# meg89/bevfusion_multimodal_3d_object_detection

Hardware: AMD Instinct MI355X
Metric: BEV frames/sec (6-cam+LiDAR, 128x128 BEV) (higher is better)
Workload: dtype fp32; 1 GPU; camera+LiDAR, 6x900x1600 images + 35k-point sweep, BEV 128x128; batch_per_gpu=8, parallelism=replicas x1, conv_kernels=wino, weights=random-init (synthetic, seeded), launch=eager, mode=inference forward -> 5 head tensors

## Files before the change

bevfusion_multimodal_3d_object_detection_amd/csrc/conv_split.hip:

```cpp
#include "conv_common.h"

#include <cmath>

namespace {

typedef __bf16 bf16x4 __attribute__((ext_vector_type(4)));
typedef unsigned u32x2 __attribute__((ext_vector_type(2)));

__device__ __forceinline__ void split3(const f32x4 v, u32x2& hi, u32x2& mid, u32x2& lo) {
  const bf16x4 h = __builtin_convertvector(v, bf16x4);
  const f32x4 r1 = v - __builtin_convertvector(h, f32x4);
  const bf16x4 m = __builtin_convertvector(r1, bf16x4);
  const f32x4 r2 = r1 - __builtin_convertvector(m, f32x4);
  const bf16x4 l = __builtin_convertvector(r2, bf16x4);
  hi = __builtin_bit_cast(u32x2, h);
  mid = __builtin_bit_cast(u32x2, m);
  lo = __builtin_bit_cast(u32x2, l);
}

__global__ __launch_bounds__(256) void split_weights(const float* __restrict__ w, __bf16* __restrict__ out, long long n) {
  const long long i = blockIdx.x * 256ll + threadIdx.x;
  if (i >= n) return;
  const float x = w[i];
  const __bf16 h = (__bf16)x;
  const float r1 = x - (float)h;
  const __bf16 m = (__bf16)r1;
  const float r2 = r1 - (float)m;
  out[i] = h;
  out[n + i] = m;
  out[2 * n + i] = (__bf16)r2;
}

template <int BM, int BN, int WM, int WN>
__device__ __forceinline__ void bound_epilogue(const ConvArgs& p, f32x16 (&acc)[WM / 32][WN / 32], const int m0, const int n0,
                                               const int m_hi, const int wm, const int wn, const int lane, const float* norms) {
  constexpr int MI = WM / 32, NI = WN / 32;
  const int h = lane >> 5, l31 = lane & 31;
  const int row_base = wm * WM + 4 * h, n_base = n0 + wn * WN;
  const int group = m0 / p.rows_per_group;
  const bool fast = (m0 + BM <= m_hi) && ((m0 + BM - 1) / p.rows_per_group == group);
  float na[MI][16];
#pragma unroll
  for (int mi = 0; mi < MI; ++mi)
#pragma unroll
    for (int r = 0; r < 16; ++r) na[mi][r] = norms[row_base + mi * 32 + (r & 3) + 8 * (r >> 2)];
  unsigned fmask[MI];
#pragma unroll
  for (int mi = 0; mi < MI; ++mi) fmask[mi] = 0u;
#pragma unroll
  for (int ni = 0; ni < NI; ++ni) {
    const int n = n_base + ni * 32 + l31;
    const bool nok = n < p.Cout;
    const int nc = nok ? n : p.Cout - 1;
    float sc, sh;
    conv_scale_shift(p, nc, sc, sh);
    const float g = p.bound_g[nc];
    const float thr = fast ? __uint_as_float(__hip_atomic_load(&p.colmax[(size_t)group * p.Cout + nc], __ATOMIC_RELAXED, __HIP_MEMORY_SCOPE_AGENT)) : 0.f;
    float lbmax = 0.f;
#pragma unroll
    for (int mi = 0; mi < MI; ++mi) {
#pragma unroll
      for (int r = 0; r < 16; ++r) {
        const float val = fmaf(acc[mi][ni][r], sc, sh);
        const float eps = fmaf(na[mi][r], g, fabsf(val) * 0x1p-21f);
        const float ub = val + eps;
        const float lb = fabsf(val) < __builtin_inff() ? val - eps : 0.f;
        if (fast) {
          lbmax = fmaxf(lbmax, lb);
          if (p.flag && !(ub < thr) && !(ub <= 0.f)) fmask[mi] |= 1u << r;
        } else {
          const int m = m0 + row_base + mi * 32 + (r & 3) + 8 * (r >> 2);
          if (m < m_hi && nok) {
            uint32_t* const t = &p.colmax[(size_t)(m / p.rows_per_group) * p.Cout + n];
            const float th = __uint_as_float(__hip_atomic_load(t, __ATOMIC_RELAXED, __HIP_MEMORY_SCOPE_AGENT));
            if (lb > th) atomicMax(t, __float_as_uint(lb));
            if (p.flag && !(ub < th) && !(ub <= 0.f)) fmask[mi] |= 1u << r;
          }
        }
      }
    }
    if (fast) {
      lbmax = fmaxf(lbmax, __shfl_xor(lbmax, 32));
      if (h == 0 && nok && lbmax > thr) atomicMax(&p.colmax[(size_t)group * p.Cout + n], __float_as_uint(lbmax));
    }
  }
  if (!p.flag) return;
#pragma unroll
  for (int mi = 0; mi < MI; ++mi) {
    unsigned f = fmask[mi];
#pragma unroll
    for (int d = 1; d < 32; d <<= 1) f |= (unsigned)__shfl_xor((int)f, d);
    const int m = m0 + row_base + mi * 32 + (l31 & 3) + 8 * ((l31 >> 2) & 3);
    if (l31 < 16 && ((f >> l31) & 1u) && m < m_hi) p.flag[m] = 1;
  }
}

template <int BM, int BN, int WM, int WN, int NPL = 3, bool BOUND = false>
__global__ __launch_bounds__(256) void conv_split(const ConvArgs p) {
  static_assert(NPL == 3 || (NPL == 2 && BOUND), "two planes are the bound pass");
  constexpr int WAVES_N = BN / WN;
  constexpr int MI = WM / 32, NI = WN / 32;
  constexpr int AP = BM / 32, BPJ = BN / 64;
  static_assert((BM / WM) * (BN / WN) == 4, "4 waves per workgroup");
  constexpr int A_PLANE = BM * 64, B_PLANE = BN * 64, B_BASE = NPL * A_PLANE;
  extern __shared__ __attribute__((aligned(16))) float lds[];
  char* const ldsb = reinterpret_cast<char*>(lds);

  const int sid = xcd_remap(blockIdx.x, gridDim.x);
  const int tm = (sid / p.tilesN) * (BOUND ? p.tm_stride : 1), tn = sid % p.tilesN;
  const int m_hi = p.M;
  const int tid = threadIdx.x, lane = tid & 63;
  const int wave = __builtin_amdgcn_readfirstlane(tid >> 6);
  const int wm = wave / WAVES_N, wn = wave % WAVES_N;
  const int m0 = tm * BM, n0 = tn * BN;

  const int chunk = tid & 7, srow = tid >> 3;
  ConvAWalker<4, AP> aw;
  aw.init(p, m0 + srow, m_hi, chunk);
  const int bq = tid & 3, brow = tid >> 2;
  unsigned b_voff[BPJ];
#pragma unroll
  for (int j = 0; j < BPJ; ++j) {
    const int n = n0 + brow + 64 * j;
    b_voff[j] = n < p.Cout ? (unsigned)(((size_t)n * p.K) * 2 + bq * 16) : kOob;
  }
  const size_t plane_elems = (size_t)p.Cout * p.K;
  const __bf16* const wb = static_cast<const __bf16*>(p.w);
  const __amdgpu_buffer_rsrc_t rsrcB0 = buf_rsrc(wb), rsrcB1 = buf_rsrc(wb + plane_elems), rsrcB2 = buf_rsrc(wb + 2 * plane_elems);

  f32x4 ra[AP];
  u32x4 rb[NPL][BPJ];
  float ssq[AP];
#pragma unroll
  for (int j = 0; j < AP; ++j) ssq[j] = 0.f;
  auto load_tile = [&](int kstep) {
    aw.load(p, ra);
#pragma unroll
    for (int j = 0; j < BPJ; ++j) {
      rb[0][j] = __builtin_amdgcn_raw_buffer_load_b128(rsrcB0, b_voff[j], (unsigned)kstep * 64u, 0);
      rb[1][j] = __builtin_amdgcn_raw_buffer_load_b128(rsrcB1, b_voff[j], (unsigned)kstep * 64u, 0);
      if constexpr (NPL == 3) rb[2][j] = __builtin_amdgcn_raw_buffer_load_b128(rsrcB2, b_voff[j], (unsigned)kstep * 64u, 0);
    }
  };

  const int a_wr = srow * 64 + (((chunk >> 1) ^ ((srow >> 1) & 3)) << 4) + (chunk & 1) * 8;
  const int b_wr = B_BASE + brow * 64 + ((bq ^ ((brow >> 1) & 3)) << 4);
  const int h = lane >> 5, l31 = lane & 31;
  int a_rd[2], b_rd[2];
#pragma unroll
  for (int g = 0; g < 2; ++g) {
    a_rd[g] = (wm * WM + l31) * 64 + (((2 * g + h) ^ ((l31 >> 1) & 3)) << 4);
    b_rd[g] = B_BASE + (wn * WN + l31) * 64 + (((2 * g + h) ^ ((l31 >> 1) & 3)) << 4);
  }
  auto store_tile = [&]() {
#pragma unroll
    for (int j = 0; j < AP; ++j) {
      u32x2 hi, mid, lo;
      split3(ra[j], hi, mid, lo);
      *reinterpret_cast<u32x2*>(ldsb + a_wr + j * 2048) = hi;
      *reinterpret_cast<u32x2*>(ldsb + a_wr + j * 2048 + A_PLANE) = mid;
      if constexpr (NPL == 3) *reinterpret_cast<u32x2*>(ldsb + a_wr + j * 2048 + 2 * A_PLANE) = lo;
      if constexpr (BOUND) ssq[j] = fmaf(ra[j][0], ra[j][0], fmaf(ra[j][1], ra[j][1], fmaf(ra[j][2], ra[j][2], fmaf(ra[j][3], ra[j][3], ssq[j]))));
    }
#pragma unroll
    for (int pl = 0; pl < NPL; ++pl)
#pragma unroll
      for (int j = 0; j < BPJ; ++j) *reinterpret_cast<u32x4*>(ldsb + b_wr + pl * B_PLANE + j * 4096) = rb[pl][j];
  };

  f32x16 acc[MI][NI];
  const f32x16 zero = {0.f, 0.f, 0.f, 0.f, 0.f, 0.f, 0.f, 0.f, 0.f, 0.f, 0.f, 0.f, 0.f, 0.f, 0.f, 0.f};
  auto compute = [&](auto firstc) {
    constexpr bool first = decltype(firstc)::value;
#pragma unroll
    for (int g = 0; g < 2; ++g) {
      bf16x8 a[NPL][MI], b[NPL][NI];
#pragma unroll
      for (int pl = 0; pl < NPL; ++pl) {
#pragma unroll
        for (int mi = 0; mi < MI; ++mi)
          a[pl][mi] = *reinterpret_cast<const bf16x8*>(ldsb + a_rd[g] + pl * A_PLANE + mi * 2048);
#pragma unroll
        for (int ni = 0; ni < NI; ++ni)
          b[pl][ni] = *reinterpret_cast<const bf16x8*>(ldsb + b_rd[g] + pl * B_PLANE + ni * 2048);
      }
      constexpr int PA[6] = {0, 2, 1, 0, 1, 0}, PB[6] = {2, 0, 1, 1, 0, 0};
      constexpr int T0 = NPL == 3 ? 0 : 3;
#pragma unroll
      for (int t = T0; t < 6; ++t)
#pragma unroll
        for (int mi = 0; mi < MI; ++mi)
#pragma unroll
          for (int ni = 0; ni < NI; ++ni)
            acc[mi][ni] = __builtin_amdgcn_mfma_f32_32x32x16_bf16(a[PA[t]][mi], b[PB[t]][ni],
                                                                  first && g == 0 && t == T0 ? zero : acc[mi][ni], 0, 0, 0);
    }
  };

  const int KT = p.K / BK;
  load_tile(0);
  store_tile();
  __syncthreads();
  if (KT > 1) {
    aw.advance(p);
    load_tile(1);
  }
  __builtin_amdgcn_sched_barrier(0);
  compute(std::true_type{});
  for (int kt = 1; kt < KT; ++kt) {
    __syncthreads();
    store_tile();
    __syncthreads();
    if (kt + 1 < KT) {
      aw.advance(p);
      load_tile(kt + 1);
    }
    __builtin_amdgcn_sched_barrier(0);
    compute(std::false_type{});
  }
  if constexpr (BOUND) {
    __syncthreads();
#pragma unroll
    for (int j = 0; j < AP; ++j) {
      float s = ssq[j];
      s += __shfl_xor(s, 1);
      s += __shfl_xor(s, 2);
      s += __shfl_xor(s, 4);
      if (chunk == 0) lds[srow + 32 * j] = fmaf(sqrtf(s), 1.f + 0x1p-10f, 0x1p-58f);
    }
    __syncthreads();
    bound_epilogue<BM, BN, WM, WN>(p, acc, m0, n0, m_hi, wm, wn, lane, lds);
  } else {
    conv_epilogue<float, BM, BN, WM, WN>(p, acc, m0, n0, m_hi, wm, wn, lane);
  }
}

template <int BM, int BN, int WM, int WN>
int launch_split(ConvArgs a, hipStream_t st) {
  a.tilesM = (a.M + BM - 1) / BM;
  a.tilesN = (a.Cout + BN - 1) / BN;
  constexpr size_t lds_bytes = size_t(3) * (BM + BN) * 64;
  return bevf_launch("bevf_conv2d_nhwc_f32x3", conv_split<BM, BN, WM, WN>, dim3(a.tilesM * a.tilesN), dim3(256), lds_bytes, st, a);
}

template <int BM, int BN, int WM, int WN>
int launch_bound(ConvArgs a, int seed_stride, hipStream_t st) {
  const int tilesM = (a.M + BM - 1) / BM;
  a.tm_stride = seed_stride > 0 ? seed_stride : 1;
  a.tilesM = (tilesM + a.tm_stride - 1) / a.tm_stride;
  a.tilesN = (a.Cout + BN - 1) / BN;
  constexpr size_t lds_bytes = size_t(2) * (BM + BN) * 64;
  return bevf_launch("bevf_conv2d_bound_f32x2", conv_split<BM, BN, WM, WN, 2, true>, dim3(a.tilesM * a.tilesN), dim3(256), lds_bytes, st, a);
}

}

extern "C" int bevf_conv2d_bound_f32x2(const bevf_conv_desc* d, const float* bound_g, int32_t* flag, int seed_stride, void* stream) {
  ConvArgs a;
  if (const int rc = conv_args_from_desc(d, "conv bound", 4, 2, &a)) return rc;
  BEVF_REQUIRE(d->colmax && bound_g && d->rows_per_group > 0 && d->relu, "conv bound: needs thresholds (colmax), bound_g, rows_per_group > 0 and relu");
  BEVF_REQUIRE(!d->y && !d->res, "conv bound: stores no y and takes no residual");
  BEVF_REQUIRE((flag != nullptr) != (seed_stride > 0), "conv bound: a seed launch (seed_stride > 0) writes no flags, a main launch (0) needs them");
  BEVF_REQUIRE(((size_t)d->Cout * d->KH * d->KW * d->Cin * 2) % 16 == 0, "conv bound: plane size must be a multiple of 16 bytes");
  a.bound_g = bound_g;
  a.flag = flag;
  hipStream_t st = static_cast<hipStream_t>(stream);
  switch (d->tile) {
    case 0: break;
    case 1: return launch_bound<128, 128, 64, 64>(a, seed_stride, st);
    case 4: return launch_bound<64, 64, 32, 32>(a, seed_stride, st);
    default: bevf_set_error("conv bound: unknown tile variant %d", d->tile); return BEVF_ERR_ARG;
  }
  if (d->Cout > 64 && a.M >= 4096) return launch_bound<128, 128, 64, 64>(a, seed_stride, st);
  return launch_bound<64, 64, 32, 32>(a, seed_stride, st);
}

extern "C" int bevf_split_weights_f32x3(const float* w, void* planes, size_t n, void* stream) {
  BEVF_REQUIRE(w && planes && n > 0, "split_weights: bad arguments");
  hipLaunchKernelGGL(split_weights, dim3((unsigned)((n + 255) / 256)), dim3(256), 0, static_cast<hipStream_t>(stream), w,
                     static_cast<__bf16*>(planes), (long long)n);
  return bevf_check_launch("bevf_split_weights_f32x3");
}

extern "C" int bevf_conv2d_nhwc_f32x3(const bevf_conv_desc* d, void* stream) {
  ConvArgs a;
  if (const int rc = conv_args_from_desc(d, "conv f32x3", 4, 2, &a)) return rc;
  BEVF_REQUIRE(d->y || d->colmax, "conv f32x3: needs y or colmax");
  BEVF_REQUIRE(!d->colmax || (d->rows_per_group > 0 && d->relu), "conv f32x3: colmax needs rows_per_group > 0 and relu (the max is taken over max(v, 0))");
  BEVF_REQUIRE(d->y_cs >= d->Cout, "conv f32x3: y_cs=%d < Cout=%d", d->y_cs, d->Cout);
  BEVF_REQUIRE(((size_t)d->Cout * d->KH * d->KW * d->Cin * 2) % 16 == 0, "conv f32x3: plane size must be a multiple of 16 bytes");
  const long long M = a.M;
  hipStream_t st = static_cast<hipStream_t>(stream);
  switch (d->tile) {
    case 0: break;
    case 1: return launch_split<128, 128, 64, 64>(a, st);
    case 3: return launch_split<128, 64, 64, 32>(a, st);
    case 4: return launch_split<64, 64, 32, 32>(a, st);
    default: bevf_set_error("conv f32x3: unknown tile variant %d", d->tile); return BEVF_ERR_ARG;
  }
  const double wg128 = std::ceil(M / 128.0) * ((d->Cout + 127) / 128);
  if (d->Cout > 64 && wg128 >= 768) return launch_split<128, 128, 64, 64>(a, st);
  if (std::ceil(M / 128.0) * ((d->Cout + 63) / 64) >= 1024) return launch_split<128, 64, 64, 32>(a, st);
  return launch_split<64, 64, 32, 32>(a, st);
}
```

Before: 295.4 frames/s.

## Double-buffer LDS and interleave staging with MFMA in bound conv pass

For the two-plane bound pass, the kernel now keeps two LDS stages and two register sets. It issues global loads two k-steps ahead and interleaves the bf16 split and LDS stores for the next tile, plus the second fragment reads, between MFMA instructions. The goal is to hide global and LDS latency and drop one barrier per k-step. It also changes the LDS swizzle pattern, requests two workgroups per CU via launch bounds, and specialises the bound epilogue on the fast and flag cases at compile time. In exchange it doubles LDS use and raises register pressure, which could limit occupancy or cause spills.

```diff
diff --git a/bevfusion_multimodal_3d_object_detection_amd/csrc/conv_split.hip b/bevfusion_multimodal_3d_object_detection_amd/csrc/conv_split.hip
--- a/bevfusion_multimodal_3d_object_detection_amd/csrc/conv_split.hip
+++ b/bevfusion_multimodal_3d_object_detection_amd/csrc/conv_split.hip
@@ -47,43 +47,50 @@
   unsigned fmask[MI];
 #pragma unroll
   for (int mi = 0; mi < MI; ++mi) fmask[mi] = 0u;
-#pragma unroll
-  for (int ni = 0; ni < NI; ++ni) {
-    const int n = n_base + ni * 32 + l31;
-    const bool nok = n < p.Cout;
-    const int nc = nok ? n : p.Cout - 1;
-    float sc, sh;
-    conv_scale_shift(p, nc, sc, sh);
-    const float g = p.bound_g[nc];
-    const float thr = fast ? __uint_as_float(__hip_atomic_load(&p.colmax[(size_t)group * p.Cout + nc], __ATOMIC_RELAXED, __HIP_MEMORY_SCOPE_AGENT)) : 0.f;
-    float lbmax = 0.f;
-#pragma unroll
-    for (int mi = 0; mi < MI; ++mi) {
-#pragma unroll
-      for (int r = 0; r < 16; ++r) {
-        const float val = fmaf(acc[mi][ni][r], sc, sh);
-        const float eps = fmaf(na[mi][r], g, fabsf(val) * 0x1p-21f);
-        const float ub = val + eps;
-        const float lb = fabsf(val) < __builtin_inff() ? val - eps : 0.f;
-        if (fast) {
-          lbmax = fmaxf(lbmax, lb);
-          if (p.flag && !(ub < thr) && !(ub <= 0.f)) fmask[mi] |= 1u << r;
-        } else {
-          const int m = m0 + row_base + mi * 32 + (r & 3) + 8 * (r >> 2);
-          if (m < m_hi && nok) {
-            uint32_t* const t = &p.colmax[(size_t)(m / p.rows_per_group) * p.Cout + n];
-            const float th = __uint_as_float(__hip_atomic_load(t, __ATOMIC_RELAXED, __HIP_MEMORY_SCOPE_AGENT));
-            if (lb > th) atomicMax(t, __float_as_uint(lb));
-            if (p.flag && !(ub < th) && !(ub <= 0.f)) fmask[mi] |= 1u << r;
+  auto run = [&](auto fastc, auto flagc) {
+    constexpr bool FAST = decltype(fastc)::value, FLAG = decltype(flagc)::value;
+#pragma unroll
+    for (int ni = 0; ni < NI; ++ni) {
+      const int n = n_base + ni * 32 + l31;
+      const bool nok = n < p.Cout;
+      const int nc = nok ? n : p.Cout - 1;
+      float sc, sh;
+      conv_scale_shift(p, nc, sc, sh);
+      const float g = p.bound_g[nc];
+      const float thr = FAST ? __uint_as_float(__hip_atomic_load(&p.colmax[(size_t)group * p.Cout + nc], __ATOMIC_RELAXED, __HIP_MEMORY_SCOPE_AGENT)) : 0.f;
+      float lbmax = 0.f;
+#pragma unroll
+      for (int mi = 0; mi < MI; ++mi) {
+#pragma unroll
+        for (int r = 0; r < 16; ++r) {
+          const float val = fmaf(acc[mi][ni][r], sc, sh);
+          const float eps = fmaf(na[mi][r], g, fabsf(val) * 0x1p-21f);
+          const float ub = val + eps;
+          const float lb = fabsf(val) < __builtin_inff() ? val - eps : 0.f;
+          if constexpr (FAST) {
+            lbmax = fmaxf(lbmax, lb);
+            if (FLAG && !(ub < thr) && !(ub <= 0.f)) fmask[mi] |= 1u << r;
+          } else {
+            const int m = m0 + row_base + mi * 32 + (r & 3) + 8 * (r >> 2);
+            if (m < m_hi && nok) {
+              uint32_t* const t = &p.colmax[(size_t)(m / p.rows_per_group) * p.Cout + n];
+              const float th = __uint_as_float(__hip_atomic_load(t, __ATOMIC_RELAXED, __HIP_MEMORY_SCOPE_AGENT));
+              if (lb > th) atomicMax(t, __float_as_uint(lb));
+              if (FLAG && !(ub < th) && !(ub <= 0.f)) fmask[mi] |= 1u << r;
+            }
           }
         }
       }
-    }
-    if (fast) {
-      lbmax = fmaxf(lbmax, __shfl_xor(lbmax, 32));
-      if (h == 0 && nok && lbmax > thr) atomicMax(&p.colmax[(size_t)group * p.Cout + n], __float_as_uint(lbmax));
-    }
-  }
+      if constexpr (FAST) {
+        lbmax = fmaxf(lbmax, __shfl_xor(lbmax, 32));
+        if (h == 0 && nok && lbmax > thr) atomicMax(&p.colmax[(size_t)group * p.Cout + n], __float_as_uint(lbmax));
+      }
+    }
+  };
+  using TT = std::true_type;
+  using FF = std::false_type;
+  if (fast) { if (p.flag) run(TT{}, TT{}); else run(TT{}, FF{}); }
+  else      { if (p.flag) run(FF{}, TT{}); else run(FF{}, FF{}); }
   if (!p.flag) return;
 #pragma unroll
   for (int mi = 0; mi < MI; ++mi) {
@@ -95,14 +102,16 @@
   }
 }
 
-template <int BM, int BN, int WM, int WN, int NPL = 3, bool BOUND = false>
-__global__ __launch_bounds__(256) void conv_split(const ConvArgs p) {
+template <int BM, int BN, int WM, int WN, int NPL = 3, bool BOUND = false, bool PIPE = BOUND>
+__global__ __launch_bounds__(256, PIPE ? 2 : 1) void conv_split(const ConvArgs p) {
   static_assert(NPL == 3 || (NPL == 2 && BOUND), "two planes are the bound pass");
   constexpr int WAVES_N = BN / WN;
   constexpr int MI = WM / 32, NI = WN / 32;
   constexpr int AP = BM / 32, BPJ = BN / 64;
   static_assert((BM / WM) * (BN / WN) == 4, "4 waves per workgroup");
   constexpr int A_PLANE = BM * 64, B_PLANE = BN * 64, B_BASE = NPL * A_PLANE;
+  constexpr int STAGE = NPL * (A_PLANE + B_PLANE);
+  constexpr int NSET = PIPE ? 2 : 1;
   extern __shared__ __attribute__((aligned(16))) float lds[];
   char* const ldsb = reinterpret_cast<char*>(lds);
 
@@ -128,95 +137,172 @@
   const __bf16* const wb = static_cast<const __bf16*>(p.w);
   const __amdgpu_buffer_rsrc_t rsrcB0 = buf_rsrc(wb), rsrcB1 = buf_rsrc(wb + plane_elems), rsrcB2 = buf_rsrc(wb + 2 * plane_elems);
 
-  f32x4 ra[AP];
-  u32x4 rb[NPL][BPJ];
+  f32x4 ra[NSET][AP];
+  u32x4 rb[NSET][NPL][BPJ];
   float ssq[AP];
 #pragma unroll
   for (int j = 0; j < AP; ++j) ssq[j] = 0.f;
-  auto load_tile = [&](int kstep) {
-    aw.load(p, ra);
+  auto load_tile = [&](auto sc, int kstep) {
+    constexpr int s = decltype(sc)::value;
+    aw.load(p, ra[s]);
 #pragma unroll
     for (int j = 0; j < BPJ; ++j) {
-      rb[0][j] = __builtin_amdgcn_raw_buffer_load_b128(rsrcB0, b_voff[j], (unsigned)kstep * 64u, 0);
-      rb[1][j] = __builtin_amdgcn_raw_buffer_load_b128(rsrcB1, b_voff[j], (unsigned)kstep * 64u, 0);
-      if constexpr (NPL == 3) rb[2][j] = __builtin_amdgcn_raw_buffer_load_b128(rsrcB2, b_voff[j], (unsigned)kstep * 64u, 0);
-    }
-  };
-
-  const int a_wr = srow * 64 + (((chunk >> 1) ^ ((srow >> 1) & 3)) << 4) + (chunk & 1) * 8;
-  const int b_wr = B_BASE + brow * 64 + ((bq ^ ((brow >> 1) & 3)) << 4);
+      rb[s][0][j] = __builtin_amdgcn_raw_buffer_load_b128(rsrcB0, b_voff[j], (unsigned)kstep * 64u, 0);
+      rb[s][1][j] = __builtin_amdgcn_raw_buffer_load_b128(rsrcB1, b_voff[j], (unsigned)kstep * 64u, 0);
+      if constexpr (NPL == 3) rb[s][2][j] = __builtin_amdgcn_raw_buffer_load_b128(rsrcB2, b_voff[j], (unsigned)kstep * 64u, 0);
+    }
+  };
+
+  const int a_wr = srow * 64 + (((chunk >> 1) ^ ((srow >> 2) & 3)) << 4) + (chunk & 1) * 8;
+  const int b_wr = B_BASE + brow * 64 + ((bq ^ ((brow >> 2) & 3)) << 4);
   const int h = lane >> 5, l31 = lane & 31;
   int a_rd[2], b_rd[2];
 #pragma unroll
   for (int g = 0; g < 2; ++g) {
-    a_rd[g] = (wm * WM + l31) * 64 + (((2 * g + h) ^ ((l31 >> 1) & 3)) << 4);
-    b_rd[g] = B_BASE + (wn * WN + l31) * 64 + (((2 * g + h) ^ ((l31 >> 1) & 3)) << 4);
-  }
-  auto store_tile = [&]() {
-#pragma unroll
-    for (int j = 0; j < AP; ++j) {
-      u32x2 hi, mid, lo;
-      split3(ra[j], hi, mid, lo);
-      *reinterpret_cast<u32x2*>(ldsb + a_wr + j * 2048) = hi;
-      *reinterpret_cast<u32x2*>(ldsb + a_wr + j * 2048 + A_PLANE) = mid;
-      if constexpr (NPL == 3) *reinterpret_cast<u32x2*>(ldsb + a_wr + j * 2048 + 2 * A_PLANE) = lo;
-      if constexpr (BOUND) ssq[j] = fmaf(ra[j][0], ra[j][0], fmaf(ra[j][1], ra[j][1], fmaf(ra[j][2], ra[j][2], fmaf(ra[j][3], ra[j][3], ssq[j]))));
-    }
-#pragma unroll
-    for (int pl = 0; pl < NPL; ++pl)
-#pragma unroll
-      for (int j = 0; j < BPJ; ++j) *reinterpret_cast<u32x4*>(ldsb + b_wr + pl * B_PLANE + j * 4096) = rb[pl][j];
+    a_rd[g] = (wm * WM + l31) * 64 + (((2 * g + h) ^ ((l31 >> 2) & 3)) << 4);
+    b_rd[g] = B_BASE + (wn * WN + l31) * 64 + (((2 * g + h) ^ ((l31 >> 2) & 3)) << 4);
+  }
+  constexpr int NPC = 2 * AP + NPL * BPJ;
+  bf16x4 ahi[AP];
+  auto stage_piece = [&](auto sc, auto pc, const int off) {
+    constexpr int s = decltype(sc)::value, i = decltype(pc)::value;
+    if constexpr (i < 2 * AP) {
+      constexpr int j = i / 2;
+      char* const dst = ldsb + off + a_wr + j * 2048;
+      const f32x4 v = ra[s][j];
+      if constexpr (i % 2 == 0) {
+        ahi[j] = __builtin_convertvector(v, bf16x4);
+        *reinterpret_cast<u32x2*>(dst) = __builtin_bit_cast(u32x2, ahi[j]);
+        if constexpr (BOUND) ssq[j] = fmaf(v[0], v[0], fmaf(v[1], v[1], fmaf(v[2], v[2], fmaf(v[3], v[3], ssq[j]))));
+      } else {
+        const f32x4 r1 = v - __builtin_convertvector(ahi[j], f32x4);
+        const bf16x4 m = __builtin_convertvector(r1, bf16x4);
+        *reinterpret_cast<u32x2*>(dst + A_PLANE) = __builtin_bit_cast(u32x2, m);
+        if constexpr (NPL == 3) {
+          const f32x4 r2 = r1 - __builtin_convertvector(m, f32x4);
+          *reinterpret_cast<u32x2*>(dst + 2 * A_PLANE) = __builtin_bit_cast(u32x2, __builtin_convertvector(r2, bf16x4));
+        }
+      }
+    } else {
+      constexpr int pl = (i - 2 * AP) / BPJ, j = (i - 2 * AP) % BPJ;
+      *reinterpret_cast<u32x4*>(ldsb + off + b_wr + pl * B_PLANE + j * 4096) = rb[s][pl][j];
+    }
+  };
+  auto store_tile = [&](auto sc, const int off) { static_for<NPC>([&](auto pc) { stage_piece(sc, pc, off); }); };
+
+  constexpr int PA[6] = {0, 2, 1, 0, 1, 0}, PB[6] = {2, 0, 1, 1, 0, 0};
+  constexpr int RA[3] = {0, NPL == 3 ? 2 : 1, 1}, RB[3] = {NPL == 3 ? 2 : 1, 0, 1};
+  constexpr int T0 = NPL == 3 ? 0 : 3, NM = 2 * (6 - T0) * MI * NI;
+  constexpr int RD_AFTER[6] = {0, 1, NPL == 3 ? 3 : 2, NPL == 3 ? 4 : 2, 5, 5};
+  auto read_part = [&](auto gc, auto kc, const int off, bf16x8 (&a)[NPL][MI], bf16x8 (&b)[NPL][NI]) {
+    constexpr int g = decltype(gc)::value, k = decltype(kc)::value, pl = k % 2 ? RB[k / 2] : RA[k / 2];
+    if constexpr (k % 2 == 0) {
+#pragma unroll
+      for (int mi = 0; mi < MI; ++mi) a[pl][mi] = *reinterpret_cast<const bf16x8*>(ldsb + off + a_rd[g] + pl * A_PLANE + mi * 2048);
+    } else {
+#pragma unroll
+      for (int ni = 0; ni < NI; ++ni) b[pl][ni] = *reinterpret_cast<const bf16x8*>(ldsb + off + b_rd[g] + pl * B_PLANE + ni * 2048);
+    }
+  };
+  auto read_frags = [&](auto gc, const int off, bf16x8 (&a)[NPL][MI], bf16x8 (&b)[NPL][NI]) {
+    static_for<2 * NPL>([&](auto kc) { read_part(gc, kc, off, a, b); });
   };
 
   f32x16 acc[MI][NI];
   const f32x16 zero = {0.f, 0.f, 0.f, 0.f, 0.f, 0.f, 0.f, 0.f, 0.f, 0.f, 0.f, 0.f, 0.f, 0.f, 0.f, 0.f};
-  auto compute = [&](auto firstc) {
-    constexpr bool first = decltype(firstc)::value;
-#pragma unroll
-    for (int g = 0; g < 2; ++g) {
-      bf16x8 a[NPL][MI], b[NPL][NI];
-#pragma unroll
-      for (int pl = 0; pl < NPL; ++pl) {
-#pragma unroll
-        for (int mi = 0; mi < MI; ++mi)
-          a[pl][mi] = *reinterpret_cast<const bf16x8*>(ldsb + a_rd[g] + pl * A_PLANE + mi * 2048);
-#pragma unroll
-        for (int ni = 0; ni < NI; ++ni)
-          b[pl][ni] = *reinterpret_cast<const bf16x8*>(ldsb + b_rd[g] + pl * B_PLANE + ni * 2048);
-      }
-      constexpr int PA[6] = {0, 2, 1, 0, 1, 0}, PB[6] = {2, 0, 1, 1, 0, 0};
-      constexpr int T0 = NPL == 3 ? 0 : 3;
-#pragma unroll
-      for (int t = T0; t < 6; ++t)
-#pragma unroll
-        for (int mi = 0; mi < MI; ++mi)
-#pragma unroll
-          for (int ni = 0; ni < NI; ++ni)
-            acc[mi][ni] = __builtin_amdgcn_mfma_f32_32x32x16_bf16(a[PA[t]][mi], b[PB[t]][ni],
-                                                                  first && g == 0 && t == T0 ? zero : acc[mi][ni], 0, 0, 0);
-    }
-  };
-
   const int KT = p.K / BK;
-  load_tile(0);
-  store_tile();
-  __syncthreads();
-  if (KT > 1) {
-    aw.advance(p);
-    load_tile(1);
-  }
-  __builtin_amdgcn_sched_barrier(0);
-  compute(std::true_type{});
-  for (int kt = 1; kt < KT; ++kt) {
+  if constexpr (PIPE) {
+#pragma unroll
+    for (int mi = 0; mi < MI; ++mi)
+#pragma unroll
+      for (int ni = 0; ni < NI; ++ni) acc[mi][ni] = zero;
+    auto step = [&](auto curc, auto stc, auto ldc, const int kt) {
+      constexpr int cur = decltype(curc)::value;
+      constexpr bool ST = decltype(stc)::value, LD = decltype(ldc)::value;
+      if constexpr (LD) {
+        aw.advance(p);
+        load_tile(ic<cur>{}, kt + 2);
+      }
+      __builtin_amdgcn_sched_barrier(0);
+      bf16x8 a[2][NPL][MI], b[2][NPL][NI];
+      read_frags(ic<0>{}, cur * STAGE, a[0], b[0]);
+      static_for<NM>([&](auto mc) {
+        constexpr int m = decltype(mc)::value;
+        constexpr int g = m / (NM / 2), t = T0 + m / (MI * NI) % (6 - T0), mi = m / NI % MI, ni = m % NI;
+        acc[mi][ni] = __builtin_amdgcn_mfma_f32_32x32x16_bf16(a[g][PA[t]][mi], b[g][PB[t]][ni], acc[mi][ni], 0, 0, 0);
+        constexpr bool rd = g == 0 && m % (MI * NI) == MI * NI - 1;
+        if constexpr (rd)
+          static_for<2 * NPL>([&](auto kc) {
+            if constexpr (RD_AFTER[decltype(kc)::value] == t - T0) read_part(ic<1>{}, kc, cur * STAGE, a[1], b[1]);
+          });
+        if constexpr (ST)
+          static_for<NPC>([&](auto pc) {
+            if constexpr (decltype(pc)::value * NM / NPC == m) stage_piece(ic<cur ^ 1>{}, pc, (cur ^ 1) * STAGE);
+          });
+        if constexpr (rd || (ST && (m * NPC + NM - 1) / NM != ((m + 1) * NPC + NM - 1) / NM)) __builtin_amdgcn_sched_barrier(0);
+      });
+      __syncthreads();
+    };
+    using TT = std::true_type;
+    using FF = std::false_type;
+    load_tile(ic<0>{}, 0);
+    store_tile(ic<0>{}, 0);
+    if (KT > 1) {
+      aw.advance(p);
+      load_tile(ic<1>{}, 1);
+    }
     __syncthreads();
-    store_tile();
+    int kt = 0;
+    for (; kt + 3 < KT; kt += 2) {
+      step(ic<0>{}, TT{}, TT{}, kt);
+      step(ic<1>{}, TT{}, TT{}, kt + 1);
+    }
+    if (KT - kt == 3) {
+      step(ic<0>{}, TT{}, TT{}, kt);
+      step(ic<1>{}, TT{}, FF{}, kt + 1);
+      step(ic<0>{}, FF{}, FF{}, kt + 2);
+    } else if (KT - kt == 2) {
+      step(ic<0>{}, TT{}, FF{}, kt);
+      step(ic<1>{}, FF{}, FF{}, kt + 1);
+    } else {
+      step(ic<0>{}, FF{}, FF{}, kt);
+    }
+  } else {
+    auto compute = [&](auto firstc) {
+      constexpr bool first = decltype(firstc)::value;
+      static_for<2>([&](auto gc) {
+        bf16x8 a[NPL][MI], b[NPL][NI];
+        read_frags(gc, 0, a, b);
+#pragma unroll
+        for (int t = T0; t < 6; ++t)
+#pragma unroll
+          for (int mi = 0; mi < MI; ++mi)
+#pragma unroll
+            for (int ni = 0; ni < NI; ++ni)
+              acc[mi][ni] = __builtin_amdgcn_mfma_f32_32x32x16_bf16(
+                  a[PA[t]][mi], b[PB[t]][ni], first && decltype(gc)::value == 0 && t == T0 ? zero : acc[mi][ni], 0, 0, 0);
+      });
+    };
+    load_tile(ic<0>{}, 0);
+    store_tile(ic<0>{}, 0);
     __syncthreads();
-    if (kt + 1 < KT) {
+    if (KT > 1) {
       aw.advance(p);
-      load_tile(kt + 1);
+      load_tile(ic<0>{}, 1);
     }
     __builtin_amdgcn_sched_barrier(0);
-    compute(std::false_type{});
+    compute(std::true_type{});
+    for (int kt = 1; kt < KT; ++kt) {
+      __syncthreads();
+      store_tile(ic<0>{}, 0);
+      __syncthreads();
+      if (kt + 1 < KT) {
+        aw.advance(p);
+        load_tile(ic<0>{}, kt + 1);
+      }
+      __builtin_amdgcn_sched_barrier(0);
+      compute(std::false_type{});
+    }
   }
   if constexpr (BOUND) {
     __syncthreads();
@@ -249,7 +335,7 @@
   a.tm_stride = seed_stride > 0 ? seed_stride : 1;
   a.tilesM = (tilesM + a.tm_stride - 1) / a.tm_stride;
   a.tilesN = (a.Cout + BN - 1) / BN;
-  constexpr size_t lds_bytes = size_t(2) * (BM + BN) * 64;
+  constexpr size_t lds_bytes = size_t(2) * 2 * (BM + BN) * 64;
   return bevf_launch("bevf_conv2d_bound_f32x2", conv_split<BM, BN, WM, WN, 2, true>, dim3(a.tilesM * a.tilesN), dim3(256), lds_bytes, st, a);
 }
 
```

Result: no change. 295.4 frames/s (-0.0%).
